# ColinWine/Multi-modal-Multi-label-Facial-Action-Unit-Detection-with-Transformer

Measured on AMD Instinct MI355X. Metric: clips/sec (fwd+bwd) on synthetic (B,T,d) AV sequences, higher is better.
Workload: dtype bf16; 1 GPU; BASELINE.json configs[1]: avformer transformer stack d=512 L=6 H=8x64 mlp=1024, T_v=196+T_a=128 tokens, B=32/GPU; global_batch=32, seq_len=324, parallelism=dp1, step=zero_grad+fwd+AULoss+bwd+adam, optimizer=FusedAdam, residual_stream=bf16

## Files before the change

multi-modal-multi-label-facial-action-unit-detection-with-transformer_amd/csrc/attn_bwd_merged.hip:

```cpp
#include <type_traits>

#include "attn_dispatch.hpp"

namespace avf {

namespace {

typedef __attribute__((ext_vector_type(16))) float f32x16_t;
typedef __attribute__((ext_vector_type(8))) short m_s16x8_t;
typedef __attribute__((ext_vector_type(4))) uint32_t m_u32x4_t;
typedef __attribute__((address_space(3))) char m_lds_char;

#ifndef AVF_PHASE_MARK
#define AVF_PHASE_INIT()
#define AVF_PHASE_MARK(slot)
#define AVF_PHASE_FLUSH()
#endif

#ifndef AVF_M4_MAXKB
#define AVF_M4_MAXKB 4
#endif

constexpr float kLog2E = 1.4426950408889634f;

#define AVF_MFMA32(a, b, c) __builtin_amdgcn_mfma_f32_32x32x16_bf16((a), (b), (c), 0, 0, 0)
#define AVF_MFMA16(a, b, c) __builtin_amdgcn_mfma_f32_16x16x32_bf16((a), (b), (c), 0, 0, 0)
#define AVF_FENCE() __builtin_amdgcn_sched_barrier(0)

__device__ __forceinline__ void m_mfma_acc(f32x16_t& acc, const bf16x8_t& a, const bf16x8_t& b) {
  asm volatile("v_mfma_f32_32x32x16_bf16 %0, %1, %2, %0" : "+a"(acc) : "v"(a), "v"(b));
}
__device__ __forceinline__ void m_operand_settle() { asm volatile("s_nop 1"); }

__device__ __forceinline__ int m_swz(int row) { return (((row >> 1) & 1) << 2) | (((row >> 2) & 1) << 1) | ((row >> 3) & 1); }
__device__ __forceinline__ int m_txor(int key) { return (((key >> 2) & 1) << 2) | (((key >> 1) & 1) << 1) | ((key >> 3) & 1); }

__device__ __forceinline__ void m_glds16(const void* g, char* l) {
  const uint32_t la = __builtin_amdgcn_readfirstlane((uint32_t)(uintptr_t)(m_lds_char*)l);
  uint32_t keep;
  asm volatile("s_mov_b32 %0, m0\n\ts_mov_b32 m0, %1\n\ts_nop 0\n\tglobal_load_lds_dwordx4 %2, off\n\ts_mov_b32 m0, %0"
               : "=&s"(keep)
               : "s"(la), "v"(g)
               : "memory");
}

__device__ __forceinline__ bf16x8_t m_row_frag(const char* p) { return *reinterpret_cast<const bf16x8_t*>(p); }

__device__ __forceinline__ bf16x8_t m_tr_frag(const char* p0, const char* p1) {
  s16x4_t lo = __builtin_amdgcn_ds_read_tr16_b64_v4i16((__attribute__((address_space(3))) s16x4_t*)(const m_lds_char*)p0);
  s16x4_t hi = __builtin_amdgcn_ds_read_tr16_b64_v4i16((__attribute__((address_space(3))) s16x4_t*)(const m_lds_char*)p1);
  m_s16x8_t r = {lo[0], lo[1], lo[2], lo[3], hi[0], hi[1], hi[2], hi[3]};
  return __builtin_bit_cast(bf16x8_t, r);
}

__device__ __forceinline__ float m_dot8(const uint4& x, const uint4& y) {
  const uint32_t a[4] = {x.x, x.y, x.z, x.w}, b[4] = {y.x, y.y, y.z, y.w};
  float acc = 0.f;
#pragma unroll
  for (int i = 0; i < 4; ++i) {
    acc = fmaf(__uint_as_float(a[i] << 16), __uint_as_float(b[i] << 16), acc);
    acc = fmaf(__uint_as_float(a[i] & 0xffff0000u), __uint_as_float(b[i] & 0xffff0000u), acc);
  }
  return acc;
}

__device__ __forceinline__ float m_sum8(float v) {
  v += AVF_DPP_F32(v, 0xB1);
  v += AVF_DPP_F32(v, 0x4E);
  v += AVF_DPP_F32(v, 0x104);
  return v;
}

__device__ __forceinline__ f32x16_t m_zero16() {
  f32x16_t z;
#pragma unroll
  for (int i = 0; i < 16; ++i) z[i] = 0.f;
  return z;
}

struct MLayout {
  int kimg, ring, nl, nd, t, total;
  __host__ __device__ MLayout(int KB, int NS) {
    kimg = 0;
    ring = kimg + 4 * KB * 32 * 128;
    nl = ring + 2 * 8192;
    nd = nl + NS * 32 * 4;
    t = nd + NS * 32 * 4;
    total = t + 2 * 4 * KB * 2048;
  }
};

template <int KB, bool RAGGED, bool MASKED = false, bool MXO = false>
__global__ __launch_bounds__(256) void attn_bwd_m4_kernel(const bf16* __restrict__ qkv, const bf16* __restrict__ o,
                                                          const bf16* __restrict__ d_o, const float* __restrict__ lse2,
                                                          bf16* __restrict__ dqkv, int N, int H,
                                                          const uint8_t* __restrict__ keep = nullptr,
                                                          uint8_t* __restrict__ dq_q = nullptr,
                                                          uint8_t* __restrict__ dq_s = nullptr) {
  constexpr int DH = 64;
  constexpr int NKB = 4 * KB;
#ifdef AVF_MXO_NO_DQ
  constexpr bool MXQ = false;
#else
  constexpr bool MXQ = MXO;
#endif
#ifdef AVF_MXO_NO_DKV
  constexpr bool MXK = false;
#else
  constexpr bool MXK = MXO;
#endif
  extern __shared__ __attribute__((aligned(16))) char m_smem[];
  const int tid = threadIdx.x, lane = tid & 63;
  const int wave = __builtin_amdgcn_readfirstlane(tid >> 6);
  const int r = lane & 31, hf = lane >> 5;
  const int bh = blockIdx.x, b = bh / H, h = bh - b * H;
  const int I = H * DH;
  const int64_t ld = 3 * (int64_t)I;
  const bf16* qbase = qkv + (int64_t)b * N * ld + h * DH;
  const bf16* kbase = qbase + I;
  const bf16* vbase = qbase + 2 * I;
  const bf16* gbase = d_o + (int64_t)b * N * I + h * DH;
  const bf16* obase = o + (int64_t)b * N * I + h * DH;
  const int NS = (N + 31) >> 5;
  const MLayout L(KB, NS);
  char* kimg = m_smem + L.kimg;
  char* ring = m_smem + L.ring;
  float* NLs = reinterpret_cast<float*>(m_smem + L.nl);
  float* NDs = reinterpret_cast<float*>(m_smem + L.nd);
  char* tbuf = m_smem + L.t;
  const int kb0 = wave * KB;

  int off_row[4];
#pragma unroll
  for (int ks = 0; ks < 4; ++ks) off_row[ks] = r * 128 + (((2 * ks + hf) ^ m_swz(r)) << 4);
  const int li = lane & 15, G = lane >> 4, gg = G & 1, qq = li >> 2, p = li & 3;
  int off_tra[2][2];
#pragma unroll
  for (int db = 0; db < 2; ++db) {
    const int ch = 4 * db + 2 * gg + (p >> 1), byte = (p & 1) * 8;
    const int ra = 4 * hf + qq;
    off_tra[db][0] = ra * 128 + ((ch ^ m_swz(ra)) << 4) + byte;
    off_tra[db][1] = (ra + 8) * 128 + ((ch ^ m_swz(ra + 8)) << 4) + byte;
  }
  int off_kq[2], off_kq2[2], off_tq[2][2];
  {
    const int rk = 4 * G + qq;
    const int ch = (MXQ ? 4 * (wave >> 1) : 2 * wave) + (p >> 1), byte = (p & 1) * 8;
    off_kq[0] = rk * 128 + ((ch ^ m_swz(rk)) << 4) + byte;
    off_kq[1] = (rk + 16) * 128 + ((ch ^ m_swz(rk + 16)) << 4) + byte;
    off_kq2[0] = rk * 128 + (((ch + 2) ^ m_swz(rk)) << 4) + byte;
    off_kq2[1] = (rk + 16) * 128 + (((ch + 2) ^ m_swz(rk + 16)) << 4) + byte;
#pragma unroll
    for (int qt = 0; qt < 2; ++qt) {
      off_tq[qt][0] = rk * 64 + (((4 * qt + p) ^ m_txor(rk)) << 3);
      off_tq[qt][1] = (rk + 16) * 64 + (((4 * qt + p) ^ m_txor(rk + 16)) << 3);
    }
  }
  int off_tw[4];
#pragma unroll
  for (int g = 0; g < 4; ++g) off_tw[g] = r * 64 + (((2 * g + hf) ^ m_txor(r)) << 3);

  AVF_PHASE_INIT();
  const int lrow = lane >> 3, lslot = lane & 7;
  for (int pc = wave; pc < 16 * KB; pc += 4) {
    const int row = pc * 8 + lrow;
    const int src = row < N ? row : N - 1;
    m_glds16(kbase + (int64_t)src * ld + ((lslot ^ m_swz(row)) << 3), kimg + pc * 1024);
  }
  auto issue_slice = [&](int s) {
    char* slot = ring + (s & 1) * 8192;
    const int lr = 8 * wave + lrow;
    int row = 32 * s + lr;
    row = row < N ? row : N - 1;
    const int ch = (lslot ^ m_swz(lr)) << 3;
    m_glds16(qbase + (int64_t)row * ld + ch, slot + wave * 1024);
    m_glds16(gbase + (int64_t)row * I + ch, slot + 4096 + wave * 1024);
  };
  issue_slice(0);
  bf16x8_t vfr[KB][4];
#pragma unroll
  for (int j = 0; j < KB; ++j)
#pragma unroll
    for (int ks = 0; ks < 4; ++ks) {
      const int key = 32 * (kb0 + j) + r;
      uint4 v = make_uint4(0, 0, 0, 0);
      if (key < N) v = *reinterpret_cast<const uint4*>(vbase + (int64_t)key * ld + 16 * ks + 8 * hf);
      vfr[j][ks] = __builtin_bit_cast(bf16x8_t, v);
    }
  for (int q = tid; q < NS * 32; q += 256) NLs[q] = q < N ? -lse2[(int64_t)bh * N + q] : -3.0e38f;
  const int drow = tid >> 3, dch = tid & 7;
  {
    float part = 0.f;
    if (drow < N) {
      const uint4 ov = *reinterpret_cast<const uint4*>(obase + (int64_t)drow * I + dch * 8);
      const uint4 gv = *reinterpret_cast<const uint4*>(gbase + (int64_t)drow * I + dch * 8);
      part = m_dot8(ov, gv);
    }
    part = m_sum8(part);
    if (dch == 0) NDs[drow] = -part;
  }
  bool kk[KB];
  uint32_t qf = 1u, qm = 0xffffffffu;
  const float dropv = -log2f((float)N);
#pragma unroll
  for (int j = 0; j < KB; ++j) kk[j] = true;
  if constexpr (MASKED) {
#pragma unroll
    for (int j = 0; j < KB; ++j) {
      const int key = 32 * (kb0 + j) + r;
      kk[j] = key < N ? keep[(int64_t)b * N + key] != 0 : false;
    }
    qf = r < N ? keep[(int64_t)b * N + r] : 1u;
  }
  __builtin_amdgcn_s_waitcnt(0x0F70);
  asm volatile("s_waitcnt vmcnt(0)" ::: "memory");
  __syncthreads();
  if (N < NKB * 32) {
    for (int idx = N * 8 + tid; idx < NKB * 32 * 8; idx += 256)
      *reinterpret_cast<uint4*>(kimg + idx * 16) = make_uint4(0, 0, 0, 0);
    __syncthreads();
  }

  AVF_PHASE_MARK(0);
  f32x16_t dkacc[KB][2], dvacc[KB][2];
#pragma unroll
  for (int j = 0; j < KB; ++j)
#pragma unroll
    for (int db = 0; db < 2; ++db) {
      dkacc[j][db] = m_zero16();
      dvacc[j][db] = m_zero16();
    }
  const float qscale = 0.125f;

  const char *qsl = nullptr, *gsl = nullptr;
  char* tcur = nullptr;
  int kopq = 0;
  bf16x8_t qa[4], ga[4], kf[4];
  f32x16_t sacc, pacc;
  m_u32x4_t pk[2], dk[2];

  bf16x8_t nlA, ndA;
  const bf16x8_t onesB = __builtin_bit_cast(bf16x8_t, m_u32x4_t{hf ? 0u : 0x3F803F80u, hf ? 0u : 0x00003F80u, 0u, 0u});
  auto split3 = [&](float x) {
    const float hi = __uint_as_float(__float_as_uint(x) & 0xffff0000u);
    const float r1 = x - hi;
    const float mid = __uint_as_float(__float_as_uint(r1) & 0xffff0000u);
    const float lo = r1 - mid;
    const uint32_t w0 = (__float_as_uint(hi) >> 16) | (__float_as_uint(mid) & 0xffff0000u);
    const uint32_t w1 = pack_bf16x2(lo, 0.f);
    return __builtin_bit_cast(bf16x8_t, m_u32x4_t{hf ? 0u : w0, hf ? 0u : w1, 0u, 0u});
  };
  auto load_kf = [&](int j) {
    const char* kblk = kimg + (kb0 + j) * 4096 + kopq;
#pragma unroll
    for (int ks = 0; ks < 4; ++ks) kf[ks] = m_row_frag(kblk + off_row[ks]);
  };
  auto stage_a = [&](auto jtag) {
    constexpr int j = decltype(jtag)::value;
    sacc = AVF_MFMA32(qa[0], kf[0], m_zero16());
    pacc = AVF_MFMA32(ga[0], vfr[j][0], m_zero16());
#pragma unroll
    for (int ks = 1; ks < 4; ++ks) {
      sacc = AVF_MFMA32(qa[ks], kf[ks], sacc);
      pacc = AVF_MFMA32(ga[ks], vfr[j][ks], pacc);
    }
    sacc = AVF_MFMA32(nlA, onesB, sacc);
    pacc = AVF_MFMA32(ndA, onesB, pacc);
    if constexpr (RAGGED && !MASKED) {
      if (32 * (kb0 + j) + 32 > N) {
        const bool dead = 32 * (kb0 + j) + r >= N;
#pragma unroll
        for (int i = 0; i < 16; ++i) sacc[i] = dead ? -INFINITY : sacc[i];
      }
    }
    if constexpr (MASKED) {
      const bool real = 32 * (kb0 + j) + r < N;
#pragma unroll
      for (int i = 0; i < 16; ++i) {
        const bool qkept = ((qm >> (8 * (i >> 2) + (i & 3))) & 1u) != 0;
        sacc[i] = qkept ? (kk[j] ? sacc[i] : -INFINITY) : (real ? dropv : -INFINITY);
      }
    }
  };
  auto b_chunk = [&](int c, m_u32x4_t (&pkn)[2], m_u32x4_t (&dkn)[2]) {
    const float p0 = __builtin_amdgcn_exp2f(sacc[2 * c]), p1 = __builtin_amdgcn_exp2f(sacc[2 * c + 1]);
    float d0 = p0 * pacc[2 * c], d1 = p1 * pacc[2 * c + 1];
    if constexpr (MASKED) {
      d0 = ((qm >> (8 * ((2 * c) >> 2) + ((2 * c) & 3))) & 1u) ? d0 : 0.f;
      d1 = ((qm >> (8 * ((2 * c + 1) >> 2) + ((2 * c + 1) & 3))) & 1u) ? d1 : 0.f;
    }
    pkn[c >> 2][c & 3] = pack_bf16x2(p0, p1);
    dkn[c >> 2][c & 3] = pack_bf16x2(d0, d1);
  };
  auto write_t = [&](auto jtag, const m_u32x4_t (&d)[2]) {
    constexpr int j = decltype(jtag)::value;
    char* timg = tcur + j * 2048;
#pragma unroll
    for (int s2 = 0; s2 < 2; ++s2) {
      *reinterpret_cast<uint2*>(timg + off_tw[2 * s2]) = make_uint2(d[s2][0], d[s2][1]);
      *reinterpret_cast<uint2*>(timg + off_tw[2 * s2 + 1]) = make_uint2(d[s2][2], d[s2][3]);
    }
  };
  auto tr_qg = [&](int db, int s2, bf16x8_t& gt, bf16x8_t& qt) {
    gt = m_tr_frag(gsl + s2 * 2048 + off_tra[db][0], gsl + s2 * 2048 + off_tra[db][1]);
    qt = m_tr_frag(qsl + s2 * 2048 + off_tra[db][0], qsl + s2 * 2048 + off_tra[db][1]);
  };
  bf16x8_t cg0, cq0, cg1, cq1;
  auto prefetch_c = [&]() { tr_qg(0, 0, cg0, cq0); tr_qg(0, 1, cg1, cq1); };
  auto phase_c = [&](auto jtag) {
    constexpr int j = decltype(jtag)::value;
    constexpr bool NX = j + 1 < KB, NX2 = j + 2 < KB;
    bf16x8_t g0, q0, g1, q1;
    m_u32x4_t pkn[2], dkn[2];
    const bf16x8_t pk0 = __builtin_bit_cast(bf16x8_t, pk[0]), pk1 = __builtin_bit_cast(bf16x8_t, pk[1]);
    const bf16x8_t dk0 = __builtin_bit_cast(bf16x8_t, dk[0]), dk1 = __builtin_bit_cast(bf16x8_t, dk[1]);
    g0 = cg0; q0 = cq0; g1 = cg1; q1 = cq1;
    m_operand_settle();
    AVF_FENCE();
    if constexpr (NX2) load_kf(j + 2);
    m_mfma_acc(dvacc[j][0], g0, pk0);
    if constexpr (NX) b_chunk(0, pkn, dkn);
    AVF_FENCE();
    m_mfma_acc(dkacc[j][0], q0, dk0);
    if constexpr (NX) b_chunk(1, pkn, dkn);
    tr_qg(1, 0, g0, q0);
    AVF_FENCE();
    m_mfma_acc(dvacc[j][0], g1, pk1);
    if constexpr (NX) b_chunk(2, pkn, dkn);
    AVF_FENCE();
    m_mfma_acc(dkacc[j][0], q1, dk1);
    if constexpr (NX) b_chunk(3, pkn, dkn);
    tr_qg(1, 1, g1, q1);
    AVF_FENCE();
    m_mfma_acc(dvacc[j][1], g0, pk0);
    if constexpr (NX) b_chunk(4, pkn, dkn);
    AVF_FENCE();
    m_mfma_acc(dkacc[j][1], q0, dk0);
    if constexpr (NX) b_chunk(5, pkn, dkn);
    AVF_FENCE();
    m_mfma_acc(dvacc[j][1], g1, pk1);
    if constexpr (NX) b_chunk(6, pkn, dkn);
    AVF_FENCE();
    m_mfma_acc(dkacc[j][1], q1, dk1);
    if constexpr (NX) b_chunk(7, pkn, dkn);
    AVF_FENCE();
    if constexpr (NX) {
      write_t(std::integral_constant<int, j + 1>{}, dkn);
      pk[0] = pkn[0]; pk[1] = pkn[1]; dk[0] = dkn[0]; dk[1] = dkn[1];
    }
    AVF_FENCE();
  };
  auto dq_job = [&](int sp, auto withb_tag) {
    constexpr bool WITHB = decltype(withb_tag)::value;
    const char* tb = tbuf + (sp & 1) * (NKB * 2048);
    const char* kb = kimg + kopq;
    f32x4_t acc0 = {0.f, 0.f, 0.f, 0.f}, acc1 = {0.f, 0.f, 0.f, 0.f};
    m_u32x4_t pkn[2], dkn[2];
    const int tq0 = MXQ ? (wave & 1) : 0;
    bf16x8_t ka = m_tr_frag(kb + off_kq[0], kb + off_kq[1]);
    bf16x8_t t0 = m_tr_frag(tb + off_tq[tq0][0], tb + off_tq[tq0][1]);
    bf16x8_t t1 = MXQ ? m_tr_frag(kb + off_kq2[0], kb + off_kq2[1]) : m_tr_frag(tb + off_tq[1][0], tb + off_tq[1][1]);
#pragma unroll
    for (int kbk = 0; kbk < NKB; ++kbk) {
      AVF_FENCE();
      bf16x8_t kan = ka, t0n = t0, t1n = t1;
      if (kbk + 1 < NKB) {
        const char* kn = kb + (kbk + 1) * 4096;
        const char* tn = tb + (kbk + 1) * 2048;
        kan = m_tr_frag(kn + off_kq[0], kn + off_kq[1]);
        t0n = m_tr_frag(tn + off_tq[tq0][0], tn + off_tq[tq0][1]);
        t1n = MXQ ? m_tr_frag(kn + off_kq2[0], kn + off_kq2[1]) : m_tr_frag(tn + off_tq[1][0], tn + off_tq[1][1]);
      }
      acc0 = AVF_MFMA16(ka, t0, acc0);
      acc1 = MXQ ? AVF_MFMA16(t1, t0, acc1) : AVF_MFMA16(ka, t1, acc1);
      if constexpr (WITHB) {
#pragma unroll
        for (int c = 0; c < 8; ++c)
          if (c * NKB / 8 == kbk) b_chunk(c, pkn, dkn);
      }
      ka = kan; t0 = t0n; t1 = t1n;
    }
    AVF_FENCE();
    if constexpr (WITHB) {
      pk[0] = pkn[0]; pk[1] = pkn[1]; dk[0] = dkn[0]; dk[1] = dkn[1];
    }
    if constexpr (MXQ) {
      const int q = 32 * sp + 16 * (wave & 1) + li;
      const int colb = h * DH + 32 * (wave >> 1);
      uint32_t sw[2][2];
      float t = 0.f;
#pragma unroll
      for (int ct = 0; ct < 2; ++ct) {
        const f32x4_t a = ct ? acc1 : acc0;
        sw[ct][0] = pack_bf16x2(a[0] * qscale, a[1] * qscale);
        sw[ct][1] = pack_bf16x2(a[2] * qscale, a[3] * qscale);
        t = fmaxf(t, fmaxf(fmaxf(fabsf(__uint_as_float(sw[ct][0] << 16)), fabsf(__uint_as_float(sw[ct][0] & 0xffff0000u))),
                           fmaxf(fabsf(__uint_as_float(sw[ct][1] << 16)), fabsf(__uint_as_float(sw[ct][1] & 0xffff0000u)))));
      }
      {
        const auto x = __builtin_amdgcn_permlane32_swap(__float_as_uint(t), __float_as_uint(t), false, false);
        t = fmaxf(__uint_as_float(x[0]), __uint_as_float(x[1]));
        const auto y = __builtin_amdgcn_permlane16_swap(__float_as_uint(t), __float_as_uint(t), false, false);
        t = fmaxf(__uint_as_float(y[0]), __uint_as_float(y[1]));
      }
      float inv;
      const uint32_t sb = mx8_scale_byte(t, &inv);
      if (q < N) {
        const int64_t row = (int64_t)b * N + q;
#pragma unroll
        for (int ct = 0; ct < 2; ++ct) {
          *reinterpret_cast<uint2*>(dqkv + row * ld + colb + 16 * ct + 4 * G) = make_uint2(sw[ct][0], sw[ct][1]);
          const float v4[4] = {__uint_as_float(sw[ct][0] << 16), __uint_as_float(sw[ct][0] & 0xffff0000u),
                               __uint_as_float(sw[ct][1] << 16), __uint_as_float(sw[ct][1] & 0xffff0000u)};
          *reinterpret_cast<uint32_t*>(dq_q + row * ld + colb + 16 * ct + 4 * G) = mx8_pack4(v4, inv);
        }
        if (G == 0) dq_s[row * (ld >> 5) + (colb >> 5)] = (uint8_t)sb;
      }
    } else {
      const uint32_t a0 = pack_bf16x2(acc0[0] * qscale, acc0[1] * qscale), a1 = pack_bf16x2(acc0[2] * qscale, acc0[3] * qscale);
      const uint32_t b0 = pack_bf16x2(acc1[0] * qscale, acc1[1] * qscale), b1 = pack_bf16x2(acc1[2] * qscale, acc1[3] * qscale);
      const auto s0 = __builtin_amdgcn_permlane16_swap(a0, b0, false, false);
      const auto s1 = __builtin_amdgcn_permlane16_swap(a1, b1, false, false);
      const int q = 32 * sp + 16 * (G & 1) + li;
      if (q < N)
        *reinterpret_cast<uint4*>(dqkv + ((int64_t)b * N + q) * ld + h * DH + 16 * wave + 4 * (G & ~1)) =
            make_uint4(s0[0], s1[0], s0[1], s1[1]);
    }
  };

  for (int s = 0; s < NS; ++s) {
    qsl = ring + (s & 1) * 8192;
    gsl = qsl + 4096;
    tcur = tbuf + (s & 1) * (NKB * 2048) + kb0 * 2048;
    uint4 onext = make_uint4(0, 0, 0, 0);
    const bool more = s + 1 < NS;
    if constexpr (MASKED) {
      const uint32_t all = (uint32_t)__builtin_amdgcn_ballot_w64(qf != 0);
      qm = all >> (4 * hf);
    }
    if (more) {
      issue_slice(s + 1);
      const int q = 32 * (s + 1) + drow;
      if (q < N) onext = *reinterpret_cast<const uint4*>(obase + (int64_t)q * I + dch * 8);
      if constexpr (MASKED) {
        const int qn = 32 * (s + 1) + r;
        qf = qn < N ? keep[(int64_t)b * N + qn] : 1u;
      }
    }
    AVF_PHASE_MARK(1);

    nlA = split3(NLs[32 * s + r]);
    ndA = split3(NDs[32 * s + r]);
    kopq = 0;
    asm volatile("" : "+v"(kopq));
#pragma unroll
    for (int ks = 0; ks < 4; ++ks) {
      qa[ks] = m_row_frag(qsl + off_row[ks]);
      ga[ks] = m_row_frag(gsl + off_row[ks]);
    }
    load_kf(0);
    stage_a(std::integral_constant<int, 0>{});
    AVF_FENCE();
    if constexpr (KB > 1) load_kf(1);
    AVF_PHASE_MARK(2);
    if (s > 0) {
      dq_job(s - 1, std::true_type{});
    } else {
      m_u32x4_t pkn[2], dkn[2];
#pragma unroll
      for (int c = 0; c < 8; ++c) b_chunk(c, pkn, dkn);
      pk[0] = pkn[0]; pk[1] = pkn[1]; dk[0] = dkn[0]; dk[1] = dkn[1];
    }
    write_t(std::integral_constant<int, 0>{}, dk);
    prefetch_c();
    AVF_FENCE();
    AVF_PHASE_MARK(3);
    if constexpr (KB > 1) stage_a(std::integral_constant<int, 1>{});
    AVF_PHASE_MARK(4);
    phase_c(std::integral_constant<int, 0>{});
    AVF_PHASE_MARK(7);
    if (more) {
      asm volatile("s_waitcnt vmcnt(0)" ::: "memory");
      const char* gn = ring + ((s + 1) & 1) * 8192 + 4096;
      const uint4 gv = *reinterpret_cast<const uint4*>(gn + (drow & 31) * 128 + ((dch ^ m_swz(drow & 31)) << 4));
      float part = m_dot8(onext, gv);
      part = m_sum8(part);
      if (dch == 0) NDs[32 * (s + 1) + drow] = (32 * (s + 1) + drow < N) ? -part : 0.f;
    }
    if constexpr (KB > 1) {
      prefetch_c();
      AVF_FENCE();
      if constexpr (KB > 2) stage_a(std::integral_constant<int, 2>{});
      AVF_PHASE_MARK(4);
      phase_c(std::integral_constant<int, 1>{});
      AVF_PHASE_MARK(7);
    }
    if constexpr (KB > 2) {
      prefetch_c();
      AVF_FENCE();
      if constexpr (KB > 3) stage_a(std::integral_constant<int, 3>{});
      AVF_PHASE_MARK(4);
      phase_c(std::integral_constant<int, 2>{});
      AVF_PHASE_MARK(7);
    }
    if constexpr (KB > 3) {
      prefetch_c();
      AVF_FENCE();
      phase_c(std::integral_constant<int, 3>{});
    }
    AVF_PHASE_MARK(7);
    __syncthreads();
    AVF_PHASE_MARK(5);
  }
  kopq = 0;
  asm volatile("" : "+v"(kopq));
  dq_job(NS - 1, std::false_type{});

  asm volatile("s_nop 15\n\ts_nop 7" ::: "memory");
  const float kscale = 1.0f / kLog2E;
#pragma unroll
  for (int j = 0; j < KB; ++j) {
    const int key = 32 * (kb0 + j) + r;
#pragma unroll
    for (int which = 0; which < 2; ++which)
#pragma unroll
      for (int db = 0; db < 2; ++db) {
        uint32_t w[4][2];
#pragma unroll
        for (int g = 0; g < 4; ++g) {
          if (which) {
            w[g][0] = pack_bf16x2(dvacc[j][db][4 * g], dvacc[j][db][4 * g + 1]);
            w[g][1] = pack_bf16x2(dvacc[j][db][4 * g + 2], dvacc[j][db][4 * g + 3]);
          } else {
            w[g][0] = pack_bf16x2(dkacc[j][db][4 * g] * kscale, dkacc[j][db][4 * g + 1] * kscale);
            w[g][1] = pack_bf16x2(dkacc[j][db][4 * g + 2] * kscale, dkacc[j][db][4 * g + 3] * kscale);
          }
        }
        const auto a0 = __builtin_amdgcn_permlane32_swap(w[0][0], w[2][0], false, false);
        const auto a1 = __builtin_amdgcn_permlane32_swap(w[0][1], w[2][1], false, false);
        const auto b0 = __builtin_amdgcn_permlane32_swap(w[1][0], w[3][0], false, false);
        const auto b1 = __builtin_amdgcn_permlane32_swap(w[1][1], w[3][1], false, false);
        if (key < N) {
          bf16* out = dqkv + ((int64_t)b * N + key) * ld + (which ? 2 * I : I) + h * DH + 32 * db + 16 * hf;
          *reinterpret_cast<uint4*>(out) = make_uint4(a0[0], a1[0], a0[1], a1[1]);
          *reinterpret_cast<uint4*>(out + 8) = make_uint4(b0[0], b1[0], b0[1], b1[1]);
        }
      }
    if constexpr (MXK) {
      const int64_t row = (int64_t)b * N + (key < N ? key : N - 1);
#pragma unroll
      for (int which = 0; which < 2; ++which)
#pragma unroll
        for (int db = 0; db < 2; ++db) {
          float v[16];
          float t = 0.f;
#pragma unroll
          for (int i = 0; i < 16; i += 2) {
            const float r0 = which ? dvacc[j][db][i] : dkacc[j][db][i] * kscale;
            const float r1 = which ? dvacc[j][db][i + 1] : dkacc[j][db][i + 1] * kscale;
            const uint32_t w = pack_bf16x2(r0, r1);
            v[i] = __uint_as_float(w << 16);
            v[i + 1] = __uint_as_float(w & 0xffff0000u);
            t = fmaxf(t, fmaxf(fabsf(v[i]), fabsf(v[i + 1])));
          }
          const auto x = __builtin_amdgcn_permlane32_swap(__float_as_uint(t), __float_as_uint(t), false, false);
          t = fmaxf(__uint_as_float(x[0]), __uint_as_float(x[1]));
          float inv;
          const uint32_t sb = mx8_scale_byte(t, &inv);
          uint32_t w[4];
#pragma unroll
          for (int g = 0; g < 4; ++g) {
            const float v4[4] = {v[4 * g], v[4 * g + 1], v[4 * g + 2], v[4 * g + 3]};
            w[g] = mx8_pack4(v4, inv);
          }
          const auto s02 = __builtin_amdgcn_permlane32_swap(w[0], w[2], false, false);
          const auto s13 = __builtin_amdgcn_permlane32_swap(w[1], w[3], false, false);
          const int col = (which ? 2 * I : I) + h * DH + 32 * db;
          if (key < N) {
            *reinterpret_cast<uint4*>(dq_q + row * ld + col + 16 * hf) = make_uint4(s02[0], s02[1], s13[0], s13[1]);
            if (hf == 0) dq_s[row * (ld >> 5) + (col >> 5)] = (uint8_t)sb;
          }
        }
    }
  }
  AVF_PHASE_MARK(6);
  AVF_PHASE_FLUSH();
}

template <int KB, bool RAGGED, bool MASKED = false, bool MXO = false>
int m4_launch(const TimingScope* ts, const bf16* qkv, const bf16* o, const bf16* d_o, const float* lse2, bf16* dqkv, int B,
              int N, int H, hipStream_t s, const uint8_t* keep = nullptr, uint8_t* dq_q = nullptr, uint8_t* dq_s = nullptr) {
  static PerDeviceOnce once;
  const MLayout L(KB, (N + 31) >> 5);
  if (once.need()) {
    hipError_t e = hipFuncSetAttribute((const void*)attn_bwd_m4_kernel<KB, RAGGED, MASKED, MXO>,
                                       hipFuncAttributeMaxDynamicSharedMemorySize, 160 * 1024);
    AVF_REQUIRE(e == hipSuccess, "attn_bwd_m4: cannot raise dynamic LDS limit: %s", hipGetErrorString(e));
    once.mark();
  }
  AVF_REQUIRE(L.total <= 160 * 1024, "attn_bwd_m4: %d bytes of LDS", L.total);
  launch_in_scope(ts, attn_bwd_m4_kernel<KB, RAGGED, MASKED, MXO>, dim3(B * H), dim3(256), (uint32_t)L.total, s, qkv, o, d_o, lse2,
                  dqkv, N, H, keep, dq_q, dq_s);
  return check_launch("attn_bwd_m4_kernel");
}

template <typename F>
int with_key_blocks(int KB, int N, F&& f) {
  switch (KB) {
    case 1: return f(int_c<1>{});
    case 2: return f(int_c<2>{});
#if AVF_M4_MAXKB >= 3
    case 3: return f(int_c<3>{});
#endif
#if AVF_M4_MAXKB >= 4
    case 4: return f(int_c<4>{});
#endif
    default: AVF_REQUIRE(false, "attn_bwd_merged: N=%d out of range", N);
  }
}

}

bool attn_bwd_merged_ok(int N, int dh, bool q_prescaled) {
  static const int allow = tuning_int("AVF_ATTN_MERGED", 1);
  static const int min_n = tuning_int("AVF_ATTN_MERGED_MIN_N", 1);
  return allow && q_prescaled && dh == 64 && N <= 512 && N >= min_n;
}

int attn_bwd_merged(const TimingScope* ts, const bf16* qkv, const bf16* o, const bf16* d_o, const float* lse2, bf16* dqkv,
                    int B, int N, int H, hipStream_t s, const void* keep, void* dq_q, void* dq_s) {
  AVF_REQUIRE(!dq_q || (dq_s && !keep && ((uintptr_t)dq_q & 3) == 0 && (3 * H * 64) % 32 == 0),
              "attn_bwd_merged: the MX-FP8 image of dqkv needs its scale buffer, no token mask and 4-byte alignment");
  AVF_REQUIRE(((uintptr_t)qkv & 15) == 0 && ((uintptr_t)o & 15) == 0 && ((uintptr_t)d_o & 15) == 0 &&
                  ((uintptr_t)dqkv & 15) == 0,
              "attn_bwd_merged: misaligned pointers");
  const int KB = (((N + 31) >> 5) + 3) >> 2;
  const bool ragged = N != 4 * KB * 32;
  return with_key_blocks(KB, N, [&](auto kb) {
    constexpr int K = decltype(kb)::value;
    if (keep) return m4_launch<K, true, true>(ts, qkv, o, d_o, lse2, dqkv, B, N, H, s, (const uint8_t*)keep);
    return with_bool(ragged, [&](auto rg) {
      constexpr bool R = decltype(rg)::value;
      if (dq_q) return m4_launch<K, R, false, true>(ts, qkv, o, d_o, lse2, dqkv, B, N, H, s, nullptr, (uint8_t*)dq_q, (uint8_t*)dq_s);
      return m4_launch<K, R>(ts, qkv, o, d_o, lse2, dqkv, B, N, H, s);
    });
  });
}

}
```

Baseline: 18100 clips/s.

## Pipeline dQ job with register-resident K fragments and register-staged Q/dO slices

```diff
diff --git a/multi-modal-multi-label-facial-action-unit-detection-with-transformer_amd/csrc/attn_bwd_merged.hip b/multi-modal-multi-label-facial-action-unit-detection-with-transformer_amd/csrc/attn_bwd_merged.hip
--- a/multi-modal-multi-label-facial-action-unit-detection-with-transformer_amd/csrc/attn_bwd_merged.hip
+++ b/multi-modal-multi-label-facial-action-unit-detection-with-transformer_amd/csrc/attn_bwd_merged.hip
@@ -19,6 +19,25 @@
 
 #ifndef AVF_M4_MAXKB
 #define AVF_M4_MAXKB 4
+#endif
+
+#ifndef AVF_M4_REG_STAGE
+#define AVF_M4_REG_STAGE 1
+#endif
+#ifndef AVF_M4_DQ_PIPE
+#define AVF_M4_DQ_PIPE 1
+#endif
+#ifndef AVF_M4_DQ_REAL
+#define AVF_M4_DQ_REAL 1
+#endif
+#ifndef AVF_M4_DQ_KREG
+#define AVF_M4_DQ_KREG 1
+#endif
+#ifndef AVF_M4_DQ_DEPTH
+#define AVF_M4_DQ_DEPTH 2
+#endif
+#ifndef AVF_M4_DQ_HEAD
+#define AVF_M4_DQ_HEAD 4
 #endif
 
 constexpr float kLog2E = 1.4426950408889634f;
@@ -221,6 +240,24 @@
     __syncthreads();
   }
 
+  constexpr bool RSTAGE = AVF_M4_REG_STAGE && KB < 4 && !(KB == 1 && MXO);
+  constexpr bool DQPIPE = AVF_M4_DQ_PIPE && KB < 4;
+  constexpr bool KREG = DQPIPE && AVF_M4_DQ_KREG && (KB <= 2 || (KB == 3 && !MXQ && !MASKED));
+  constexpr int DQD = KREG ? AVF_M4_DQ_DEPTH : 1;
+  constexpr int DQR = DQD + 1;
+  static_assert(DQD >= 1 && DQR * (KREG ? (MXQ ? 2 : 4) : 6) <= 15, "attn_bwd_m4: dQ fragment ring deeper than lgkmcnt counts");
+  constexpr int DQH = !DQPIPE ? 0 : (AVF_M4_DQ_HEAD < NKB - 3 ? AVF_M4_DQ_HEAD : NKB - 3);
+  const int nkr = (DQPIPE && AVF_M4_DQ_REAL) ? NS : NKB;
+  bf16x8_t kaR[KREG ? NKB : 1], ka2R[KREG && MXQ ? NKB : 1];
+  if constexpr (KREG) {
+#pragma unroll
+    for (int kbk = 0; kbk < NKB; ++kbk) {
+      const char* kn = kimg + kbk * 4096;
+      kaR[kbk] = m_tr_frag(kn + off_kq[0], kn + off_kq[1]);
+      if constexpr (MXQ) ka2R[kbk] = m_tr_frag(kn + off_kq2[0], kn + off_kq2[1]);
+    }
+  }
+
   AVF_PHASE_MARK(0);
   f32x16_t dkacc[KB][2], dvacc[KB][2];
 #pragma unroll
@@ -350,13 +387,111 @@
     }
     AVF_FENCE();
   };
-  auto dq_job = [&](int sp, auto withb_tag) {
+  bf16x8_t dqa[KREG ? 1 : DQR], dqt0[DQR], dqt1[DQR];
+  f32x4_t dqacc0, dqacc1;
+  const char* dqtb = nullptr;
+  const int tq0 = MXQ ? (wave & 1) : 0;
+  auto dq_read = [&](int kbk) {
+    const int sl = kbk % DQR;
+    const char* tn = dqtb + kbk * 2048;
+    if constexpr (!KREG) {
+      const char* kn = kimg + kopq + kbk * 4096;
+      dqa[sl] = m_tr_frag(kn + off_kq[0], kn + off_kq[1]);
+      if constexpr (MXQ) dqt1[sl] = m_tr_frag(kn + off_kq2[0], kn + off_kq2[1]);
+    }
+    dqt0[sl] = m_tr_frag(tn + off_tq[tq0][0], tn + off_tq[tq0][1]);
+    if constexpr (!MXQ) dqt1[sl] = m_tr_frag(tn + off_tq[1][0], tn + off_tq[1][1]);
+  };
+  auto dq_begin = [&](int sp) {
+    dqtb = tbuf + (sp & 1) * (NKB * 2048);
+    dqacc0 = f32x4_t{0.f, 0.f, 0.f, 0.f};
+    dqacc1 = f32x4_t{0.f, 0.f, 0.f, 0.f};
+#pragma unroll
+    for (int kbk = 0; kbk < DQD && kbk < NKB; ++kbk) dq_read(kbk);
+  };
+  auto dq_blocks = [&](auto k0tag, auto k1tag, auto withb_tag) {
+    constexpr int K0 = decltype(k0tag)::value, K1 = decltype(k1tag)::value;
+    constexpr bool WITHB = decltype(withb_tag)::value;
+    m_u32x4_t pkn[2], dkn[2];
+#pragma unroll
+    for (int kbk = K0; kbk < K1; ++kbk) {
+      AVF_FENCE();
+      if (kbk + DQD < NKB) dq_read(kbk + DQD);
+      if (kbk < NKB - 3 || kbk < nkr) {
+        const int sl = kbk % DQR;
+        if constexpr (KREG) {
+          dqacc0 = AVF_MFMA16(kaR[kbk], dqt0[sl], dqacc0);
+          dqacc1 = MXQ ? AVF_MFMA16(ka2R[MXQ ? kbk : 0], dqt0[sl], dqacc1) : AVF_MFMA16(kaR[kbk], dqt1[sl], dqacc1);
+        } else {
+          dqacc0 = AVF_MFMA16(dqa[sl], dqt0[sl], dqacc0);
+          dqacc1 = MXQ ? AVF_MFMA16(dqt1[sl], dqt0[sl], dqacc1) : AVF_MFMA16(dqa[sl], dqt1[sl], dqacc1);
+        }
+      }
+      if constexpr (WITHB) {
+#pragma unroll
+        for (int c = 0; c < 8; ++c)
+          if (K0 + c * (K1 - K0) / 8 == kbk) {
+            b_chunk(c, pkn, dkn);
+            asm volatile("" : "+v"(pkn[c >> 2][c & 3]), "+v"(dkn[c >> 2][c & 3]));
+          }
+      }
+    }
+    AVF_FENCE();
+    if constexpr (WITHB) {
+      pk[0] = pkn[0]; pk[1] = pkn[1]; dk[0] = dkn[0]; dk[1] = dkn[1];
+    }
+  };
+  auto dq_store = [&](int sp) {
+    const f32x4_t acc0 = dqacc0, acc1 = dqacc1;
+    if constexpr (MXQ) {
+      const int q = 32 * sp + 16 * (wave & 1) + li;
+      const int colb = h * DH + 32 * (wave >> 1);
+      uint32_t sw[2][2];
+      float t = 0.f;
+#pragma unroll
+      for (int ct = 0; ct < 2; ++ct) {
+        const f32x4_t a = ct ? acc1 : acc0;
+        sw[ct][0] = pack_bf16x2(a[0] * qscale, a[1] * qscale);
+        sw[ct][1] = pack_bf16x2(a[2] * qscale, a[3] * qscale);
+        t = fmaxf(t, fmaxf(fmaxf(fabsf(__uint_as_float(sw[ct][0] << 16)), fabsf(__uint_as_float(sw[ct][0] & 0xffff0000u))),
+                           fmaxf(fabsf(__uint_as_float(sw[ct][1] << 16)), fabsf(__uint_as_float(sw[ct][1] & 0xffff0000u)))));
+      }
+      {
+        const auto x = __builtin_amdgcn_permlane32_swap(__float_as_uint(t), __float_as_uint(t), false, false);
+        t = fmaxf(__uint_as_float(x[0]), __uint_as_float(x[1]));
+        const auto y = __builtin_amdgcn_permlane16_swap(__float_as_uint(t), __float_as_uint(t), false, false);
+        t = fmaxf(__uint_as_float(y[0]), __uint_as_float(y[1]));
+      }
+      float inv;
+      const uint32_t sb = mx8_scale_byte(t, &inv);
+      if (q < N) {
+        const int64_t row = (int64_t)b * N + q;
+#pragma unroll
+        for (int ct = 0; ct < 2; ++ct) {
+          *reinterpret_cast<uint2*>(dqkv + row * ld + colb + 16 * ct + 4 * G) = make_uint2(sw[ct][0], sw[ct][1]);
+          const float v4[4] = {__uint_as_float(sw[ct][0] << 16), __uint_as_float(sw[ct][0] & 0xffff0000u),
+                               __uint_as_float(sw[ct][1] << 16), __uint_as_float(sw[ct][1] & 0xffff0000u)};
+          *reinterpret_cast<uint32_t*>(dq_q + row * ld + colb + 16 * ct + 4 * G) = mx8_pack4(v4, inv);
+        }
+        if (G == 0) dq_s[row * (ld >> 5) + (colb >> 5)] = (uint8_t)sb;
+      }
+    } else {
+      const uint32_t a0 = pack_bf16x2(acc0[0] * qscale, acc0[1] * qscale), a1 = pack_bf16x2(acc0[2] * qscale, acc0[3] * qscale);
+      const uint32_t b0 = pack_bf16x2(acc1[0] * qscale, acc1[1] * qscale), b1 = pack_bf16x2(acc1[2] * qscale, acc1[3] * qscale);
+      const auto s0 = __builtin_amdgcn_permlane16_swap(a0, b0, false, false);
+      const auto s1 = __builtin_amdgcn_permlane16_swap(a1, b1, false, false);
+      const int q = 32 * sp + 16 * (G & 1) + li;
+      if (q < N)
+        *reinterpret_cast<uint4*>(dqkv + ((int64_t)b * N + q) * ld + h * DH + 16 * wave + 4 * (G & ~1)) =
+            make_uint4(s0[0], s1[0], s0[1], s1[1]);
+    }
+  };
+  auto dq_job_serial = [&](int sp, auto withb_tag) {
     constexpr bool WITHB = decltype(withb_tag)::value;
     const char* tb = tbuf + (sp & 1) * (NKB * 2048);
     const char* kb = kimg + kopq;
     f32x4_t acc0 = {0.f, 0.f, 0.f, 0.f}, acc1 = {0.f, 0.f, 0.f, 0.f};
     m_u32x4_t pkn[2], dkn[2];
-    const int tq0 = MXQ ? (wave & 1) : 0;
     bf16x8_t ka = m_tr_frag(kb + off_kq[0], kb + off_kq[1]);
     bf16x8_t t0 = m_tr_frag(tb + off_tq[tq0][0], tb + off_tq[tq0][1]);
     bf16x8_t t1 = MXQ ? m_tr_frag(kb + off_kq2[0], kb + off_kq2[1]) : m_tr_frag(tb + off_tq[1][0], tb + off_tq[1][1]);
@@ -384,62 +519,30 @@
     if constexpr (WITHB) {
       pk[0] = pkn[0]; pk[1] = pkn[1]; dk[0] = dkn[0]; dk[1] = dkn[1];
     }
-    if constexpr (MXQ) {
-      const int q = 32 * sp + 16 * (wave & 1) + li;
-      const int colb = h * DH + 32 * (wave >> 1);
-      uint32_t sw[2][2];
-      float t = 0.f;
-#pragma unroll
-      for (int ct = 0; ct < 2; ++ct) {
-        const f32x4_t a = ct ? acc1 : acc0;
-        sw[ct][0] = pack_bf16x2(a[0] * qscale, a[1] * qscale);
-        sw[ct][1] = pack_bf16x2(a[2] * qscale, a[3] * qscale);
-        t = fmaxf(t, fmaxf(fmaxf(fabsf(__uint_as_float(sw[ct][0] << 16)), fabsf(__uint_as_float(sw[ct][0] & 0xffff0000u))),
-                           fmaxf(fabsf(__uint_as_float(sw[ct][1] << 16)), fabsf(__uint_as_float(sw[ct][1] & 0xffff0000u)))));
-      }
-      {
-        const auto x = __builtin_amdgcn_permlane32_swap(__float_as_uint(t), __float_as_uint(t), false, false);
-        t = fmaxf(__uint_as_float(x[0]), __uint_as_float(x[1]));
-        const auto y = __builtin_amdgcn_permlane16_swap(__float_as_uint(t), __float_as_uint(t), false, false);
-        t = fmaxf(__uint_as_float(y[0]), __uint_as_float(y[1]));
-      }
-      float inv;
-      const uint32_t sb = mx8_scale_byte(t, &inv);
-      if (q < N) {
-        const int64_t row = (int64_t)b * N + q;
-#pragma unroll
-        for (int ct = 0; ct < 2; ++ct) {
-          *reinterpret_cast<uint2*>(dqkv + row * ld + colb + 16 * ct + 4 * G) = make_uint2(sw[ct][0], sw[ct][1]);
-          const float v4[4] = {__uint_as_float(sw[ct][0] << 16), __uint_as_float(sw[ct][0] & 0xffff0000u),
-                               __uint_as_float(sw[ct][1] << 16), __uint_as_float(sw[ct][1] & 0xffff0000u)};
-          *reinterpret_cast<uint32_t*>(dq_q + row * ld + colb + 16 * ct + 4 * G) = mx8_pack4(v4, inv);
-        }
-        if (G == 0) dq_s[row * (ld >> 5) + (colb >> 5)] = (uint8_t)sb;
-      }
-    } else {
-      const uint32_t a0 = pack_bf16x2(acc0[0] * qscale, acc0[1] * qscale), a1 = pack_bf16x2(acc0[2] * qscale, acc0[3] * qscale);
-      const uint32_t b0 = pack_bf16x2(acc1[0] * qscale, acc1[1] * qscale), b1 = pack_bf16x2(acc1[2] * qscale, acc1[3] * qscale);
-      const auto s0 = __builtin_amdgcn_permlane16_swap(a0, b0, false, false);
-      const auto s1 = __builtin_amdgcn_permlane16_swap(a1, b1, false, false);
-      const int q = 32 * sp + 16 * (G & 1) + li;
-      if (q < N)
-        *reinterpret_cast<uint4*>(dqkv + ((int64_t)b * N + q) * ld + h * DH + 16 * wave + 4 * (G & ~1)) =
-            make_uint4(s0[0], s1[0], s0[1], s1[1]);
-    }
+    dqacc0 = acc0;
+    dqacc1 = acc1;
+    dq_store(sp);
   };
 
   for (int s = 0; s < NS; ++s) {
     qsl = ring + (s & 1) * 8192;
     gsl = qsl + 4096;
     tcur = tbuf + (s & 1) * (NKB * 2048) + kb0 * 2048;
-    uint4 onext = make_uint4(0, 0, 0, 0);
+    uint4 onext = make_uint4(0, 0, 0, 0), qnext = onext, gnext = onext;
     const bool more = s + 1 < NS;
     if constexpr (MASKED) {
       const uint32_t all = (uint32_t)__builtin_amdgcn_ballot_w64(qf != 0);
       qm = all >> (4 * hf);
     }
     if (more) {
-      issue_slice(s + 1);
+      if constexpr (RSTAGE) {
+        int row = 32 * (s + 1) + drow;
+        row = row < N ? row : N - 1;
+        qnext = *reinterpret_cast<const uint4*>(qbase + (int64_t)row * ld + dch * 8);
+        gnext = *reinterpret_cast<const uint4*>(gbase + (int64_t)row * I + dch * 8);
+      } else {
+        issue_slice(s + 1);
+      }
       const int q = 32 * (s + 1) + drow;
       if (q < N) onext = *reinterpret_cast<const uint4*>(obase + (int64_t)q * I + dch * 8);
       if constexpr (MASKED) {
@@ -449,8 +552,12 @@
     }
     AVF_PHASE_MARK(1);
 
-    nlA = split3(NLs[32 * s + r]);
-    ndA = split3(NDs[32 * s + r]);
+    if (DQH > 0 && s > 0) dq_begin(s - 1);
+    const float nlraw = NLs[32 * s + r], ndraw = NDs[32 * s + r];
+    if constexpr (DQH == 0) {
+      nlA = split3(nlraw);
+      ndA = split3(ndraw);
+    }
     kopq = 0;
     asm volatile("" : "+v"(kopq));
 #pragma unroll
@@ -459,12 +566,24 @@
       ga[ks] = m_row_frag(gsl + off_row[ks]);
     }
     load_kf(0);
+    if (DQH > 0 && s > 0) dq_blocks(std::integral_constant<int, 0>{}, std::integral_constant<int, DQH>{}, std::false_type{});
+    if constexpr (DQH > 0) {
+      AVF_FENCE();
+      nlA = split3(nlraw);
+      ndA = split3(ndraw);
+    }
     stage_a(std::integral_constant<int, 0>{});
     AVF_FENCE();
     if constexpr (KB > 1) load_kf(1);
     AVF_PHASE_MARK(2);
     if (s > 0) {
-      dq_job(s - 1, std::true_type{});
+      if constexpr (DQPIPE) {
+        if (DQH == 0) dq_begin(s - 1);
+        dq_blocks(std::integral_constant<int, DQH>{}, std::integral_constant<int, NKB>{}, std::true_type{});
+        dq_store(s - 1);
+      } else {
+        dq_job_serial(s - 1, std::true_type{});
+      }
     } else {
       m_u32x4_t pkn[2], dkn[2];
 #pragma unroll
@@ -480,9 +599,17 @@
     phase_c(std::integral_constant<int, 0>{});
     AVF_PHASE_MARK(7);
     if (more) {
-      asm volatile("s_waitcnt vmcnt(0)" ::: "memory");
-      const char* gn = ring + ((s + 1) & 1) * 8192 + 4096;
-      const uint4 gv = *reinterpret_cast<const uint4*>(gn + (drow & 31) * 128 + ((dch ^ m_swz(drow & 31)) << 4));
+      uint4 gv;
+      if constexpr (RSTAGE) {
+        char* dst = ring + ((s + 1) & 1) * 8192 + drow * 128 + ((dch ^ m_swz(drow)) << 4);
+        *reinterpret_cast<uint4*>(dst) = qnext;
+        *reinterpret_cast<uint4*>(dst + 4096) = gnext;
+        gv = gnext;
+      } else {
+        asm volatile("s_waitcnt vmcnt(0)" ::: "memory");
+        const char* gn = ring + ((s + 1) & 1) * 8192 + 4096;
+        gv = *reinterpret_cast<const uint4*>(gn + (drow & 31) * 128 + ((dch ^ m_swz(drow & 31)) << 4));
+      }
       float part = m_dot8(onext, gv);
       part = m_sum8(part);
       if (dch == 0) NDs[32 * (s + 1) + drow] = (32 * (s + 1) + drow < N) ? -part : 0.f;
@@ -514,7 +641,13 @@
   }
   kopq = 0;
   asm volatile("" : "+v"(kopq));
-  dq_job(NS - 1, std::false_type{});
+  if constexpr (DQPIPE) {
+    dq_begin(NS - 1);
+    dq_blocks(std::integral_constant<int, 0>{}, std::integral_constant<int, NKB>{}, std::false_type{});
+    dq_store(NS - 1);
+  } else {
+    dq_job_serial(NS - 1, std::false_type{});
+  }
 
   asm volatile("s_nop 15\n\ts_nop 7" ::: "memory");
   const float kscale = 1.0f / kLog2E;
```

Result: no change. 18110 clips/s (median of 6 runs) (+0.1%).
